# diaoenmao/HeteroFL-Computation-and-Communication-Efficient-Federated-Learning-for-Heterogeneous-Clients

Hardware: AMD Instinct MI355X
Metric: local-train samples/sec/node (higher is better)
Workload: dtype bfloat16; 1 GPU; model=resnet18, dataset=CIFAR10, control_name=1_100_0.1_iid_fix_a1-e1_bn_1_1, active_clients=10, local_epochs=5, global_batch=10, parallelism=client-dp1, engine=batched

## Files before the change

### heterofl_amd/ops/csrc/bindings.cpp

```cpp
#include <torch/extension.h>

std::vector<at::Tensor> bn_relu_fwd(at::Tensor x, at::Tensor gamma,
                                    at::Tensor beta, double eps);
std::vector<at::Tensor> bn_relu_bwd(at::Tensor dy, at::Tensor x,
                                    at::Tensor gamma, at::Tensor beta,
                                    at::Tensor mean, at::Tensor invstd);
std::vector<at::Tensor> gn_relu_fwd(at::Tensor x, at::Tensor gamma,
                                    at::Tensor beta, int64_t G, double eps);
std::vector<at::Tensor> gn_relu_bwd(at::Tensor dy, at::Tensor x,
                                    at::Tensor gamma, at::Tensor beta,
                                    at::Tensor mean, at::Tensor invstd,
                                    int64_t G);
std::vector<at::Tensor> masked_ce_fwd(at::Tensor scores, at::Tensor labels,
                                      at::Tensor mask, at::Tensor metrics);
at::Tensor masked_ce_bwd(at::Tensor scores, at::Tensor labels, at::Tensor mask,
                         at::Tensor up);
std::vector<at::Tensor> build_chunk_table(std::vector<at::Tensor> grads,
                                          std::vector<at::Tensor> params,
                                          std::vector<at::Tensor> bufs,
                                          int64_t R, int64_t chunk_elems,
                                          std::vector<at::Tensor> shadows);
void fill_chunk_table(at::Tensor blob, std::vector<at::Tensor> grads,
                      std::vector<at::Tensor> params,
                      std::vector<at::Tensor> bufs, int64_t R,
                      int64_t chunk_elems, std::vector<at::Tensor> shadows);
void clip_sgd_step(at::Tensor table_blob, int64_t n_chunks,
                   at::Tensor chunk_client, at::Tensor partials,
                   at::Tensor normsq, double max_norm, double lr,
                   double momentum, double weight_decay);
// ... 63 lines not shown
at::Tensor conv_pack_weight(at::Tensor w);
at::Tensor conv_fwd_large(at::Tensor x, at::Tensor packed, at::Tensor bias,
                          at::Tensor residual, int64_t stride, int64_t pad,
                          int64_t Cin, int64_t Cout, int64_t k);
at::Tensor bn_relu_infer(at::Tensor x, at::Tensor scale, at::Tensor shift);
std::vector<at::Tensor> eval_metrics(at::Tensor scores, at::Tensor labels,
                                     at::Tensor user_ptr,
                                     at::Tensor user_samples,
                                     at::Tensor label_mask);
at::Tensor lm_head_pack(at::Tensor w);
std::vector<at::Tensor> lm_head_ce(at::Tensor x, at::Tensor packed,
                                   at::Tensor bias, at::Tensor labels,
                                   at::Tensor vocab_mask, int64_t V,
                                   int64_t E, int64_t splits);
std::vector<at::Tensor> lm_head_topk(at::Tensor x, at::Tensor packed,
                                     at::Tensor bias, at::Tensor labels,
                                     at::Tensor vocab_mask, int64_t V,
                                     int64_t E, int64_t k, int64_t splits);
int64_t lm_head_topk_splits(int64_t M, int64_t V);

PYBIND11_MODULE(TORCH_EXTENSION_NAME, m) {
    m.def("bn_relu_fwd", &bn_relu_fwd, "fused sBN+ReLU forward");
    m.def("bn_relu_bwd", &bn_relu_bwd, "fused sBN+ReLU backward");
    m.def("gn_relu_fwd", &gn_relu_fwd, "fused GroupNorm+ReLU forward");
    m.def("gn_relu_bwd", &gn_relu_bwd, "fused GroupNorm+ReLU backward");
    m.def("masked_ce_fwd", &masked_ce_fwd, "batched masked CE forward");
    m.def("masked_ce_bwd", &masked_ce_bwd, "batched masked CE backward");
    m.def("build_chunk_table", &build_chunk_table,
          "build clip+SGD chunk table");
    m.def("clip_sgd_step", &clip_sgd_step, "fused per-client clip+SGD step");
    m.def("fill_chunk_table", &fill_chunk_table,
          "fill a preallocated chunk table post-capture");
    m.def("conv_fwd", &conv_fwd, "MFMA implicit-GEMM grouped conv forward");
    m.def("conv_bwd_data", &conv_bwd_data, "MFMA grouped conv backward-data");
    m.def("conv_bwd_weight", &conv_bwd_weight,
          "MFMA grouped conv backward-weight (fp32 out)");
    m.def("conv_plan", &conv_plan,
          "(route, split, dynamic LDS bytes) the conv launchers would take; "
          "launches nothing");
    m.def("conv_plan_variant", &conv_plan_variant,
          "name of the kernel the conv launcher would launch; launches "
          "nothing");
    m.def("mfma_probe", &mfma_probe, "16x16x32 bf16 MFMA layout probe");
    m.def("head_fwd", &head_fwd, "fused avgpool+per-client-linear forward");
    m.def("head_bwd", &head_bwd, "fused head backward");
    m.def("attn_fwd", &attn_fwd, "fused small-S attention forward");
// ... 44 lines not shown
```

### heterofl_amd/ops/csrc/clip_sgd.hip

```cpp
#include "common.h"

struct Chunk {
    const float* grad;
    float* param;
    float* buf;
    __hip_bfloat16* shadow;
    int len;
    int client;
};

__global__ void __launch_bounds__(256)
sqnorm_kernel(const Chunk* __restrict__ chunks,
              float* __restrict__ partials) {
    const Chunk ck = chunks[blockIdx.x];
    float s = 0.f;
    for (int i = threadIdx.x; i < ck.len; i += blockDim.x) {
        const float g = ck.grad[i];
        s += g * g;
    }
    __shared__ float scratch[256 / WAVE];
    for (int off = WAVE / 2; off > 0; off >>= 1) s += __shfl_down(s, off, WAVE);
    const int wid = threadIdx.x / WAVE;
    if ((threadIdx.x & (WAVE - 1)) == 0) scratch[wid] = s;
    __syncthreads();
// ... 11 lines not shown
    const int r = blockIdx.x;
    float s = 0.f;
    for (int i = threadIdx.x; i < n_chunks; i += 64)
        if (chunk_client[i] == r) s += partials[i];
    for (int off = WAVE / 2; off > 0; off >>= 1) s += __shfl_down(s, off, WAVE);
    if (threadIdx.x == 0) normsq[r] = s;
}

__global__ void __launch_bounds__(256)
clip_sgd_step_kernel(const Chunk* __restrict__ chunks,
                     const float* __restrict__ normsq, float max_norm,
                     float lr, float momentum, float weight_decay) {
    const Chunk ck = chunks[blockIdx.x];
    const float norm = sqrtf(normsq[ck.client]);
    const float scale = fminf(max_norm / (norm + 1e-6f), 1.f);
    for (int i = threadIdx.x; i < ck.len; i += blockDim.x) {
        const float p = ck.param[i];
        float g = ck.grad[i] * scale + weight_decay * p;
        const float b = momentum * ck.buf[i] + g;
        ck.buf[i] = b;
        const float pn = p - lr * b;
        ck.param[i] = pn;
        if (ck.shadow) ck.shadow[i] = __float2bfloat16(pn);
    }
}

#include <torch/extension.h>
#include <ATen/hip/HIPContext.h>

std::vector<at::Tensor> build_chunk_table(std::vector<at::Tensor> grads,
                                          std::vector<at::Tensor> params,
                                          std::vector<at::Tensor> bufs,
                                          int64_t R, int64_t chunk_elems,
                                          std::vector<at::Tensor> shadows) {
    std::vector<Chunk> host;
    for (size_t t = 0; t < grads.size(); ++t) {
        TORCH_CHECK(grads[t].is_contiguous() && params[t].is_contiguous() &&
                    bufs[t].is_contiguous());
        TORCH_CHECK(grads[t].scalar_type() == at::kFloat,
                    "clip_sgd expects fp32 master grads/params");
        const long numel = grads[t].numel();
        TORCH_CHECK(numel % R == 0);
        const long per = numel / R;
        const float* g = grads[t].data_ptr<float>();
        float* p = params[t].data_ptr<float>();
        float* b = bufs[t].data_ptr<float>();
// ... 55 lines not shown
                ck.grad = g + r * per + off;
                ck.param = p + r * per + off;
                ck.buf = b + r * per + off;
                ck.shadow = sh ? sh + r * per + off : nullptr;
                ck.len = (int)std::min((long)chunk_elems, per - off);
                ck.client = (int)r;
                host.push_back(ck);
            }
    }
    TORCH_CHECK((long)(host.size() * sizeof(Chunk)) == blob.numel(),
                "chunk table size changed");
    auto src = at::from_blob(host.data(), {(long)(host.size() * sizeof(Chunk))},
                             at::TensorOptions().dtype(at::kByte)).clone();
    blob.copy_(src, false);
}

void clip_sgd_step(at::Tensor table_blob, int64_t n_chunks,
                   at::Tensor chunk_client, at::Tensor partials,
                   at::Tensor normsq, double max_norm, double lr,
                   double momentum, double weight_decay) {
    auto stream = at::hip::getCurrentHIPStream();
    const Chunk* chunks = (const Chunk*)table_blob.data_ptr();
    const int R = (int)normsq.numel();
    hipLaunchKernelGGL(sqnorm_kernel, dim3((int)n_chunks), dim3(256), 0,
                       stream, chunks, partials.data_ptr<float>());
    hipLaunchKernelGGL(sqnorm_reduce_kernel, dim3(R), dim3(64), 0, stream,
                       partials.data_ptr<float>(),
                       chunk_client.data_ptr<int>(), (int)n_chunks,
                       normsq.data_ptr<float>());
    hipLaunchKernelGGL(clip_sgd_step_kernel, dim3((int)n_chunks), dim3(256), 0,
                       stream, chunks, normsq.data_ptr<float>(),
                       (float)max_norm, (float)lr, (float)momentum,
                       (float)weight_decay);
}
```

### heterofl_amd/ops/csrc/common.h

```cpp
#pragma once
#include <hip/hip_runtime.h>
#include <hip/hip_bf16.h>

#define WAVE 64

typedef __attribute__((ext_vector_type(4))) float f32x4;
typedef __attribute__((ext_vector_type(8))) __bf16 bf16x8;
typedef __attribute__((ext_vector_type(8))) unsigned short u16x8;

template <typename T>
__device__ __forceinline__ float ld_f32(const T* p) { return (float)*p; }
template <>
__device__ __forceinline__ float ld_f32<__hip_bfloat16>(const __hip_bfloat16* p) {
    return __bfloat162float(*p);
}

template <typename T>
__device__ __forceinline__ void st_f32(T* p, float v) { *p = (T)v; }
template <>
__device__ __forceinline__ void st_f32<__hip_bfloat16>(__hip_bfloat16* p, float v) {
    *p = __float2bfloat16(v);
}

__device__ __forceinline__ void block_reduce2(float& v1, float& v2, float* scratch) {
    for (int off = WAVE / 2; off > 0; off >>= 1) {
        v1 += __shfl_down(v1, off, WAVE);
        v2 += __shfl_down(v2, off, WAVE);
    }
    const int wid = threadIdx.x / WAVE;
    const int nw = blockDim.x / WAVE;
    if ((threadIdx.x & (WAVE - 1)) == 0) {
        scratch[2 * wid] = v1;
        scratch[2 * wid + 1] = v2;
    }
    __syncthreads();
    if (threadIdx.x < WAVE) {
        float a = (threadIdx.x < nw) ? scratch[2 * threadIdx.x] : 0.f;
        float b = (threadIdx.x < nw) ? scratch[2 * threadIdx.x + 1] : 0.f;
        for (int off = WAVE / 2; off > 0; off >>= 1) {
            a += __shfl_down(a, off, WAVE);
            b += __shfl_down(b, off, WAVE);
        }
        if (threadIdx.x == 0) { scratch[0] = a; scratch[1] = b; }
    }
// ... 6 lines not shown
```

### heterofl_amd/ops/csrc/conv_mfma.hip

```cpp
#include "common.h"

constexpr int BM = 64;
constexpr int BP = 64;
constexpr int BK = 32;
constexpr int LDK = BK + 8;

template <typename T>
__device__ __forceinline__ f32x4 mfma_tile(const T* a_row, const T* b_col,
                                           f32x4 acc);

template <>
__device__ __forceinline__ f32x4 mfma_tile<__hip_bfloat16>(
        const __hip_bfloat16* a_row, const __hip_bfloat16* b_col, f32x4 acc) {
    const int l = threadIdx.x & (WAVE - 1);
    const int kb = (l >> 4) * 8;
    bf16x8 a = *(const bf16x8*)(a_row + kb);
    bf16x8 b = *(const bf16x8*)(b_col + kb);
    return __builtin_amdgcn_mfma_f32_16x16x32_bf16(a, b, acc, 0, 0, 0);
}

template <>
__device__ __forceinline__ f32x4 mfma_tile<float>(const float* a_row,
                                                  const float* b_col,
                                                  f32x4 acc) {
// ... 227 lines not shown
            for (int r = 0; r < 4; ++r) {
                const int m = m0 + wm + fm * 16 + (l >> 4) * 4 + r;
                if (m < M && yb >= 0)
                    fwd_store(acc[fm][fp][r], yb + (long)m * OHW,
                              g * gm.Cout + m, bias, residual, y, partial,
                              slab, splitk);
            }
        }
}

template <typename T>
__global__ void __launch_bounds__(256)
conv_out_reduce_kernel(const float* __restrict__ partial,
                       const float* __restrict__ bias,
                       const T* __restrict__ residual, T* __restrict__ out,
                       long total, long chanstride, int nchan, int splitk) {
    const long i = (long)blockIdx.x * blockDim.x + threadIdx.x;
    if (i >= total) return;
    float v = 0.f;
    for (int sp = 0; sp < splitk; ++sp) v += partial[(long)sp * total + i];
    if (bias) v += bias[(i / chanstride) % nchan];
    if (residual) v += ld_f32(residual + i);
    st_f32(out + i, v);
}

template <typename T, typename TA, typename TB>
__global__ void __launch_bounds__(256)
conv_bwd_data_kernel(const T* __restrict__ dy, const float* __restrict__ w,
                     T* __restrict__ dx, float* __restrict__ partial,
                     ConvGeom gm, int splitk) {
    __shared__ TA a_lds[BM][LDK];
    __shared__ TB b_lds[BP][LDK];
    __shared__ int t_oh[BP], t_ow[BP];
    __shared__ long t_dybase[BP], t_xbase[BP];
    const TileCoord tc = tile_coord(gm.G);
    const int g = tc.g, sp = tc.sp;
    const int c0 = tc.row0, q0 = tc.col0;
    const int kk2 = gm.khw * gm.khw;
    const int J = gm.Cout * kk2;
    const int K = gm.Cin * kk2;
    const int HW = gm.H * gm.W;
    const int Q = gm.N * HW;
    const int OHW = gm.OH * gm.OW;
    const int tid = tc.tid, l = tc.l, wm = tc.wm, wp = tc.wp;

    if (tid < BP) {
// ... 333 lines not shown
    }
    float* slab = out + (long)sp * GK;
#pragma unroll
    for (int fm = 0; fm < 2; ++fm)
#pragma unroll
        for (int fp = 0; fp < 2; ++fp)
#pragma unroll
            for (int r = 0; r < 4; ++r) {
                const int m = m0 + wm + fm * 16 + (l >> 4) * 4 + r;
                const int k = k0 + wp + fp * 16 + (l & 15);
                if (m < M && k < K)
                    slab[(long)(g * gm.Cout + m) * K + k] = acc[fm][fp][r];
            }
}

__global__ void __launch_bounds__(256)
splitp_reduce_kernel(const float* __restrict__ partials,
                     float* __restrict__ dw, long GK, int splitp) {
    const long i = (long)blockIdx.x * blockDim.x + threadIdx.x;
    if (i >= GK) return;
    float s = 0.f;
    for (int sp = 0; sp < splitp; ++sp) s += partials[(long)sp * GK + i];
    dw[i] = s;
}


constexpr int WIN_CH = BK / 9 + 2;
constexpr int WIN_ROWS = 16;
constexpr int WIN_W = 40;

template <typename T, typename TA, typename TB>
__global__ void __launch_bounds__(256)
conv_fwd_staged_kernel(const T* __restrict__ x, const float* __restrict__ w,
                       const float* __restrict__ bias,
                       const T* __restrict__ residual, T* __restrict__ y,
                       float* __restrict__ partial, ConvGeom gm, int splitk) {
    __shared__ TA a_lds[BM][LDK];
    __shared__ TB b_lds[BP][LDK];
    __shared__ float win[WIN_CH][WIN_ROWS][WIN_W];
    const TileCoord tc = tile_coord(gm.G);
    const int g = tc.g, sp = tc.sp;
    const int m0 = tc.row0, p0 = tc.col0;
    const int kk2 = gm.khw * gm.khw;
    const int K = gm.Cin * kk2;
    const int M = gm.Cout;
    const int OHW = gm.OH * gm.OW;
// ... 1638 lines not shown
    std::string stem;
    if (direction == "fwd") {
        pl = plan_fwd(gm, (int)elem_size, fp8 != 0);
        stem = "conv_fwd";
    } else if (direction == "bwd_data") {
        pl = plan_bwd_data(gm, (int)elem_size, fp8 != 0);
        stem = pl.route == GATHER_S2 ? "conv_bwd_data_s2" : "conv_bwd_data";
    } else if (direction == "bwd_weight") {
        pl = plan_bwd_weight(gm, (int)elem_size, fp8 != 0);
        stem = "conv_bwd_weight";
    } else {
        TORCH_CHECK(false, "direction must be fwd, bwd_data or bwd_weight");
    }
    if (pl.route == RESIDENT) return stem + "_resident_kernel";
    if (pl.route == STAGED) return stem + "_staged_kernel";
    if (pl.tabled) return stem + "_tabled_kernel";
    return stem + (pl.fp8 ? "_kernel<fp8>" : "_kernel");
}

#define DISPATCH_CONV_FT(t, ...)                                              \
    if ((t) == at::kFloat) { using scalar_t = float; __VA_ARGS__; }           \
    else if ((t) == at::kBFloat16) { using scalar_t = __hip_bfloat16; __VA_ARGS__; } \
    else { TORCH_CHECK(false, "unsupported dtype"); }

template <typename T>
static auto fwd_kernel(const ConvPlan& pl) {
    if (pl.route == STAGED) return conv_fwd_staged_kernel<T, T, T>;
    if constexpr (std::is_same<T, __hip_bfloat16>::value)
        if (pl.fp8) return conv_fwd_kernel<T, e4m3, e4m3>;
    return conv_fwd_kernel<T, T, T>;
}
template <typename T>
static auto bwd_data_kernel(const ConvPlan& pl) {
    if (pl.route == STAGED) return conv_bwd_data_staged_kernel<T, T, T>;
    if constexpr (std::is_same<T, __hip_bfloat16>::value)
        if (pl.fp8) return conv_bwd_data_kernel<T, e4m3, e5m2>;
    return conv_bwd_data_kernel<T, T, T>;
}
template <typename T>
static auto bwd_data_s2_kernel(const ConvPlan& pl) {
    if constexpr (std::is_same<T, __hip_bfloat16>::value)
        if (pl.fp8) return conv_bwd_data_s2_kernel<T, e4m3, e5m2>;
    return conv_bwd_data_s2_kernel<T, T, T>;
}
template <typename T>
static auto bwd_weight_kernel(const ConvPlan& pl) {
// ... 29 lines not shown
                                 : nullptr;
        scalar_t* yp = (scalar_t*)y.data_ptr();
        if (pl.route == RESIDENT) {
            const int K = gm.Cin * gm.khw * gm.khw;
            const int flags =
                ((gm.W % (16 / esz) == 0 && aligned16(xp)) ? 1 : 0)
                | ((K % 4 == 0 && aligned16(wp)) ? 2 : 0);
            hipLaunchKernelGGL(conv_fwd_resident_kernel<scalar_t>, pl.grid,
                               dim3(256), pl.dyn_lds, stream, xp, wp, bp, rp,
                               yp, pp, gm, pl.split, pl.tab0, flags);
        } else if (pl.tabled) {
            const int K = gm.Cin * gm.khw * gm.khw;
            const int flags = (K % 4 == 0 && aligned16(wp)) ? 2 : 0;
            hipLaunchKernelGGL(conv_fwd_tabled_kernel<scalar_t>, pl.grid,
                               dim3(256), pl.tab_lds, stream, xp, wp, bp, rp, yp, pp,
                               gm, pl.split, flags);
        } else {
            hipLaunchKernelGGL(fwd_kernel<scalar_t>(pl), pl.grid, dim3(256),
                               0, stream, xp, wp, bp, rp, yp, pp, gm,
                               pl.split);
        }
        if (pl.split > 1) {
            const long total = y.numel();
            hipLaunchKernelGGL(conv_out_reduce_kernel<scalar_t>,
                               dim3((int)((total + 255) / 256)), dim3(256), 0,
                               stream, pp, bp, rp, yp, total,
                               (long)gm.OH * gm.OW, gm.G * gm.Cout, pl.split);
        }
    });
    return y;
}

at::Tensor conv_bwd_data(at::Tensor dy, at::Tensor w, int64_t groups,
                         int64_t stride, int64_t pad, int64_t H, int64_t W,
                         int64_t fp8) {
    TORCH_CHECK(dy.is_cuda() && w.is_contiguous());
    TORCH_CHECK(stride == 1 || stride == 2, "stride must be 1 or 2");
    auto dyc = dy.contiguous();
    const ConvGeom gm = conv_geom(groups, dy.size(0), w.size(1), H, W,
                                  w.size(0) / groups, w.size(2), stride, pad);
    TORCH_CHECK(dy.size(2) == gm.OH && dy.size(3) == gm.OW,
                "dy does not match the conv geometry");
    const int esz = (int)dy.element_size();
    const ConvPlan pl = plan_bwd_data(gm, esz, fp8 != 0);
    auto dx = at::empty({gm.N, gm.G * gm.Cin, gm.H, gm.W}, dy.options());
    at::Tensor partial;
    if (pl.split > 1)
        partial = at::empty({(long)pl.split * dx.numel()},
                            dy.options().dtype(at::kFloat));
    float* pp = pl.split > 1 ? partial.data_ptr<float>() : nullptr;
// ... 8 lines not shown
            hipLaunchKernelGGL(conv_bwd_data_resident_kernel<scalar_t>,
                               pl.grid, dim3(256), pl.dyn_lds, stream, dyp,
                               wp, dxp, pp, gm, pl.split, pl.tab0, pl.tab1,
                               flags);
        } else if (pl.tabled && pl.route == GATHER_S2) {
            hipLaunchKernelGGL(conv_bwd_data_s2_tabled_kernel<scalar_t>,
                               pl.grid, dim3(256), pl.tab_lds, stream, dyp, wp, dxp,
                               pp, gm, pl.split, pl.nyp);
        } else if (pl.tabled) {
            hipLaunchKernelGGL(conv_bwd_data_tabled_kernel<scalar_t>,
                               pl.grid, dim3(256), pl.tab_lds, stream, dyp, wp, dxp,
                               pp, gm, pl.split);
        } else if (pl.route == GATHER_S2) {
            hipLaunchKernelGGL(bwd_data_s2_kernel<scalar_t>(pl), pl.grid,
                               dim3(256), 0, stream, dyp, wp, dxp, pp, gm,
                               pl.split, pl.nyp);
        } else {
            hipLaunchKernelGGL(bwd_data_kernel<scalar_t>(pl), pl.grid,
                               dim3(256), 0, stream, dyp, wp, dxp, pp, gm,
                               pl.split);
        }
        if (pl.split > 1) {
            const long total = dx.numel();
            hipLaunchKernelGGL(conv_out_reduce_kernel<scalar_t>,
                               dim3((int)((total + 255) / 256)), dim3(256), 0,
                               stream, pp, nullptr, nullptr, dxp, total, 1L,
                               1, pl.split);
        }
    });
    return dx;
}

at::Tensor conv_bwd_weight(at::Tensor dy, at::Tensor x, int64_t groups,
                           int64_t stride, int64_t pad, int64_t khw,
                           int64_t fp8) {
    auto dyc = dy.contiguous();
    const ConvGeom gm = conv_geom(groups, x.size(0), x.size(1) / groups,
                                  x.size(2), x.size(3), dy.size(1) / groups,
                                  khw, stride, pad);
    TORCH_CHECK(dy.size(2) == gm.OH && dy.size(3) == gm.OW,
                "dy does not match the conv geometry");
    const int esz = (int)x.element_size();
    const ConvPlan pl = plan_bwd_weight(gm, esz, fp8 != 0);
    const long GK = (long)gm.G * gm.Cout * gm.Cin * gm.khw * gm.khw;
    auto dw = at::empty({(long)gm.G * gm.Cout, gm.Cin, gm.khw, gm.khw},
                        x.options().dtype(at::kFloat));
    at::Tensor partials;
    if (pl.split > 1)
        partials = at::empty({pl.split, GK}, x.options().dtype(at::kFloat));
    float* out = pl.split > 1 ? partials.data_ptr<float>()
// ... 3 lines not shown
        const scalar_t* dyp = (const scalar_t*)dyc.data_ptr();
        const scalar_t* xp = (const scalar_t*)x.data_ptr();
        if (pl.route == RESIDENT) {
            const int flags =
                ((gm.W % (16 / esz) == 0 && aligned16(xp)) ? 1 : 0)
                | (aligned16(dyp) ? 2 : 0);
            hipLaunchKernelGGL(conv_bwd_weight_resident_kernel<scalar_t>,
                               pl.grid, dim3(256), pl.dyn_lds, stream, dyp,
                               xp, out, gm, pl.split, flags);
        } else if (pl.tabled) {
            const int OHW = gm.OH * gm.OW;
            const int pchunk = cdiv(gm.N * OHW, pl.split);
            const int flags = (OHW % 8 == 0 && pchunk % 8 == 0
                               && aligned16(dyp)) ? 2 : 0;
            hipLaunchKernelGGL(conv_bwd_weight_tabled_kernel<scalar_t>,
                               pl.grid, dim3(256), 0, stream, dyp, xp, out,
                               gm, pl.split, flags);
        } else {
            hipLaunchKernelGGL(bwd_weight_kernel<scalar_t>(pl), pl.grid,
                               dim3(256), 0, stream, dyp, xp, out, gm,
                               pl.split);
        }
    });
    if (pl.split > 1)
        hipLaunchKernelGGL(splitp_reduce_kernel,
                           dim3((int)((GK + 255) / 256)), dim3(256), 0,
                           stream, out, dw.data_ptr<float>(), GK, pl.split);
    return dw;
}

__global__ void mfma_probe_kernel(const float* __restrict__ A,
                                  const float* __restrict__ B,
                                  float* __restrict__ D) {
    const int l = threadIdx.x;
    const int kb = (l >> 4) * 8;
    bf16x8 a, b;
#pragma unroll
    for (int j = 0; j < 8; ++j) {
        a[j] = (__bf16)A[(l & 15) * 32 + kb + j];
        b[j] = (__bf16)B[(kb + j) * 16 + (l & 15)];
    }
    f32x4 acc = {};
    acc = __builtin_amdgcn_mfma_f32_16x16x32_bf16(a, b, acc, 0, 0, 0);
#pragma unroll
    for (int r = 0; r < 4; ++r)
        D[((l >> 4) * 4 + r) * 16 + (l & 15)] = acc[r];
}

at::Tensor mfma_probe(at::Tensor A, at::Tensor B) {
    TORCH_CHECK(A.sizes() == at::IntArrayRef({16, 32}) &&
// ... 11 lines not shown
```

### heterofl_amd/ops/csrc/fused_norm.hip

```cpp
#include "common.h"

template <typename T, bool STAGE>
__global__ void __launch_bounds__(256)
bn_relu_fwd_kernel(const T* __restrict__ x, const float* __restrict__ gamma,
                   const float* __restrict__ beta, T* __restrict__ y,
                   float* __restrict__ mean_out, float* __restrict__ invstd_out,
                   int N, int C, int HW, float eps) {
    const int c = blockIdx.x;
    __shared__ float scratch[2 * 256 / WAVE];
    extern __shared__ __attribute__((aligned(16))) char smem[];
    T* stage = (T*)smem;
    float s1 = 0.f, s2 = 0.f;
    const long chan_off = (long)c * HW;
    const long samp_stride = (long)C * HW;
    for (int i = threadIdx.x; i < N * HW; i += blockDim.x) {
        const int n = i / HW, hw = i - n * HW;
        const T raw = x[n * samp_stride + chan_off + hw];
        if (STAGE) stage[i] = raw;
        const float v = (float)raw;
        s1 += v;
        s2 += v * v;
    }
    block_reduce2(s1, s2, scratch);
    const float inv_m = 1.f / (N * HW);
// ... 124 lines not shown
        s2 += d * xh;
    }
    block_reduce2(s1, s2, scratch);
    if (threadIdx.x == 0) {
        dbeta[c] = s1;
        dgamma[c] = s2;
    }
    const float inv_M = 1.f / (N * HW);
    const float k1 = s1 * inv_M, k2 = s2 * inv_M;
    const float gis = g * is;
    for (int i = threadIdx.x; i < N * HW; i += blockDim.x) {
        const int n = i / HW, hw = i - n * HW;
        const long off = n * samp_stride + chan_off + hw;
        float xh, d;
        if (STAGE) {
            xh = ((float)sx[i] - m) * is;
            d = (float)sd[i];
        } else {
            xh = (ld_f32(x + off) - m) * is;
            const float pre = xh * g + b;
            d = pre > 0.f ? ld_f32(dy + off) : 0.f;
        }
        st_f32(dx + off, gis * (d - k1 - xh * k2));
    }
}

template <typename T, bool STAGE>
__global__ void __launch_bounds__(256)
gn_relu_fwd_kernel(const T* __restrict__ x, const float* __restrict__ gamma,
                   const float* __restrict__ beta, T* __restrict__ y,
                   float* __restrict__ mean_out, float* __restrict__ invstd_out,
                   int N, int C, int HW, int G, float eps) {
    const int ng = blockIdx.x;
    const int n = ng / G, j = ng - n * G;
    const int cpg = C / G;
    __shared__ float scratch[2 * 256 / WAVE];
    extern __shared__ __attribute__((aligned(16))) char smem[];
    T* stage = (T*)smem;
    const long base = (long)n * C * HW + (long)j * cpg * HW;
    const int M = cpg * HW;
    float s1 = 0.f, s2 = 0.f;
    for (int i = threadIdx.x; i < M; i += blockDim.x) {
        const T raw = x[base + i];
        if (STAGE) stage[i] = raw;
        const float v = (float)raw;
        s1 += v;
// ... 61 lines not shown
        s2 += d * g * xh;
    }
    block_reduce2(s1, s2, scratch);
    const float inv_M = 1.f / M;
    const float k1 = s1 * inv_M, k2 = s2 * inv_M;
    for (int i = threadIdx.x; i < M; i += blockDim.x) {
        const int c = j * cpg + i / HW;
        const float g = gamma ? gamma[c] : 1.f;
        const float b = beta ? beta[c] : 0.f;
        const float xh = (ld_f32(x + base + i) - m) * is;
        const float pre = xh * g + b;
        const float d = pre > 0.f ? ld_f32(dy + base + i) : 0.f;
        st_f32(dx + base + i, is * (d * g - k1 - xh * k2));
    }
}

#include <torch/extension.h>
#include <ATen/hip/HIPContext.h>

#define DISPATCH_FT(t, ...)                                                   \
    if ((t) == at::kFloat) { using scalar_t = float; __VA_ARGS__; }           \
    else if ((t) == at::kBFloat16) { using scalar_t = __hip_bfloat16; __VA_ARGS__; } \
    else { TORCH_CHECK(false, "unsupported dtype"); }

std::vector<at::Tensor> bn_relu_fwd(at::Tensor x, at::Tensor gamma,
                                    at::Tensor beta, double eps) {
    TORCH_CHECK(x.is_cuda() && x.is_contiguous());
    const int N = x.size(0), C = x.size(1);
    const int HW = x.numel() / (N * C);
    auto y = at::empty_like(x);
    auto opts = x.options().dtype(at::kFloat);
    auto mean = at::empty({C}, opts);
    auto invstd = at::empty({C}, opts);
    auto stream = at::hip::getCurrentHIPStream();
    const long stage_bytes = (long)N * HW * x.element_size();
    const long M = (long)N * HW;
    if (M > 64 * 1024) {
        const int S = std::max(1, std::min(N, (4096 + C - 1) / C));
        auto partials = at::empty({(long)C * S * 2}, opts);
        auto scale_shift = at::empty({2L * C}, opts);
        DISPATCH_FT(x.scalar_type(), {
            hipLaunchKernelGGL(bn_sums_kernel<scalar_t>, dim3(C, S),
                               dim3(256), 0, stream,
                               (const scalar_t*)x.data_ptr(),
                               partials.data_ptr<float>(), N, C, HW, S);
            hipLaunchKernelGGL(bn_finalize_kernel,
                               dim3((C + 255) / 256), dim3(256), 0, stream,
                               partials.data_ptr<float>(),
                               gamma.defined() ? gamma.data_ptr<float>()
                                               : nullptr,
                               beta.defined() ? beta.data_ptr<float>()
                                              : nullptr,
                               mean.data_ptr<float>(),
                               invstd.data_ptr<float>(),
                               scale_shift.data_ptr<float>(), C, S,
                               (float)(1.0 / M), (float)eps);
            hipLaunchKernelGGL(bn_apply_relu_kernel<scalar_t>, dim3(C, S),
                               dim3(256), 0, stream,
                               (const scalar_t*)x.data_ptr(),
                               scale_shift.data_ptr<float>(),
                               (scalar_t*)y.data_ptr(), N, C, HW, S);
        });
        return {y, mean, invstd};
    }
    DISPATCH_FT(x.scalar_type(), {
        if (stage_bytes <= 64 * 1024)
            hipLaunchKernelGGL((bn_relu_fwd_kernel<scalar_t, true>), dim3(C),
                               dim3(256), (int)stage_bytes, stream,
                               (const scalar_t*)x.data_ptr(),
                               gamma.defined() ? gamma.data_ptr<float>()
                                               : nullptr,
                               beta.defined() ? beta.data_ptr<float>()
                                              : nullptr,
                               (scalar_t*)y.data_ptr(),
                               mean.data_ptr<float>(),
                               invstd.data_ptr<float>(), N, C, HW,
                               (float)eps);
        else
            hipLaunchKernelGGL((bn_relu_fwd_kernel<scalar_t, false>), dim3(C),
                               dim3(256), 0, stream,
                               (const scalar_t*)x.data_ptr(),
                               gamma.defined() ? gamma.data_ptr<float>()
                                               : nullptr,
                               beta.defined() ? beta.data_ptr<float>()
                                              : nullptr,
                               (scalar_t*)y.data_ptr(),
                               mean.data_ptr<float>(),
                               invstd.data_ptr<float>(), N, C, HW,
                               (float)eps);
    });
    return {y, mean, invstd};
}

std::vector<at::Tensor> bn_relu_bwd(at::Tensor dy, at::Tensor x,
                                    at::Tensor gamma, at::Tensor beta,
                                    at::Tensor mean, at::Tensor invstd) {
    const int N = x.size(0), C = x.size(1);
    const int HW = x.numel() / (N * C);
    auto dx = at::empty_like(x);
    auto opts = x.options().dtype(at::kFloat);
    auto dgamma = at::empty({C}, opts);
    auto dbeta = at::empty({C}, opts);
    auto dyc = dy.contiguous();
    auto stream = at::hip::getCurrentHIPStream();
    const long stage_bytes = 2L * N * (x.numel() / (N * C)) * x.element_size();
    DISPATCH_FT(x.scalar_type(), {
        if (stage_bytes <= 64 * 1024)
            hipLaunchKernelGGL((bn_relu_bwd_kernel<scalar_t, true>), dim3(C),
                               dim3(256), (int)stage_bytes, stream,
                               (const scalar_t*)dyc.data_ptr(),
                               (const scalar_t*)x.data_ptr(),
                               gamma.defined() ? gamma.data_ptr<float>()
                                               : nullptr,
                               beta.defined() ? beta.data_ptr<float>()
                                              : nullptr,
                               mean.data_ptr<float>(),
                               invstd.data_ptr<float>(),
                               (scalar_t*)dx.data_ptr(),
                               dgamma.data_ptr<float>(),
                               dbeta.data_ptr<float>(), N, C, HW);
        else
            hipLaunchKernelGGL((bn_relu_bwd_kernel<scalar_t, false>), dim3(C),
                               dim3(256), 0, stream,
                               (const scalar_t*)dyc.data_ptr(),
                               (const scalar_t*)x.data_ptr(),
                               gamma.defined() ? gamma.data_ptr<float>()
                                               : nullptr,
                               beta.defined() ? beta.data_ptr<float>()
                                              : nullptr,
                               mean.data_ptr<float>(),
                               invstd.data_ptr<float>(),
                               (scalar_t*)dx.data_ptr(),
                               dgamma.data_ptr<float>(),
                               dbeta.data_ptr<float>(), N, C, HW);
    });
    return {dx, dgamma, dbeta};
}

std::vector<at::Tensor> gn_relu_fwd(at::Tensor x, at::Tensor gamma,
                                    at::Tensor beta, int64_t G, double eps) {
    TORCH_CHECK(x.is_cuda() && x.is_contiguous());
    const int N = x.size(0), C = x.size(1);
    const int HW = x.numel() / (N * C);
    TORCH_CHECK(C % G == 0, "channels not divisible by groups");
    auto y = at::empty_like(x);
    auto opts = x.options().dtype(at::kFloat);
    auto mean = at::empty({N * G}, opts);
    auto invstd = at::empty({N * G}, opts);
    auto stream = at::hip::getCurrentHIPStream();
    const long gsb = ((long)C / G) * (x.numel() / (N * C)) * x.element_size();
    DISPATCH_FT(x.scalar_type(), {
        if (gsb <= 64 * 1024)
            hipLaunchKernelGGL((gn_relu_fwd_kernel<scalar_t, true>),
                               dim3(N * G), dim3(256), (int)gsb, stream,
                               (const scalar_t*)x.data_ptr(),
                               gamma.defined() ? gamma.data_ptr<float>()
                                               : nullptr,
// ... 68 lines not shown
```

### heterofl_amd/ops/fused.py

```python
import torch
import torch.nn.functional as F

from . import require_native, use_native, large_conv_enabled


class _FusedNormReLU(torch.autograd.Function):

    @staticmethod
    def forward(ctx, x, weight, bias, kind, groups, eps):
        ext = require_native()
        x = x.contiguous()
        if kind == 'bn':
            y, mean, invstd = ext.bn_relu_fwd(x, weight, bias, eps)
        else:
            y, mean, invstd = ext.gn_relu_fwd(x, weight, bias, groups, eps)
        ctx.save_for_backward(x, weight, bias, mean, invstd)
        ctx.kind = kind
        ctx.groups = groups
        return y

    @staticmethod
    def backward(ctx, dy):
        ext = require_native()
        x, weight, bias, mean, invstd = ctx.saved_tensors
        if ctx.kind == 'bn':
            dx, dgamma, dbeta = ext.bn_relu_bwd(dy, x, weight, bias, mean,
                                                invstd)
        else:
            dx, dgamma, dbeta = ext.gn_relu_bwd(dy, x, weight, bias, mean,
                                                invstd, ctx.groups)
        return dx, dgamma, dbeta, None, None, None


def fused_norm_relu(x, weight, bias, kind, groups=1, eps=1e-5):
    return _FusedNormReLU.apply(x, weight, bias, kind, groups, eps)


def eager_scaler_norm_relu(x, weight, bias, kind, groups, rate, eps=1e-5):
    if rate != 1.0:
        x = x / rate
    if kind == 'bn':
        x = F.batch_norm(x, None, None, weight, bias, training=True, eps=eps)
    else:
        x = F.group_norm(x, groups, weight, bias, eps=eps)
    return F.relu(x)


class _FusedMaskedCE(torch.autograd.Function):

    @staticmethod
    def forward(ctx, scores, labels, mask, metrics):
        ext = require_native()
        scores = scores.contiguous().float()
        (losses,) = ext.masked_ce_fwd(
            scores, labels.contiguous(),
            mask if mask is not None else torch.Tensor(),
            metrics if metrics is not None else torch.Tensor())
        ctx.save_for_backward(scores, labels,
# ... 571 lines not shown
```

Baseline: 24820 samples/s.

## Vectorize memory-bound streaming kernels: clip-SGD, split-K reductions, BN+ReLU

Adds 16-byte vectorized variants of several bandwidth-bound kernels: an unrolled squared-norm kernel and float4 clip+SGD step, float4 split-K output and weight-gradient reductions with fused bias and residual, and vectorized staged BN+ReLU forward/backward. A route selector picks the vector path when pointers and sizes are aligned and the HETEROFL_STREAM_VEC environment variable does not disable it. The goal is fewer memory instructions and better load-level parallelism in elementwise and reduction passes, at the cost of more code paths and alignment-dependent dispatch. A new binding reports which BN route would be taken.

```diff
diff --git a/heterofl_amd/ops/csrc/bindings.cpp b/heterofl_amd/ops/csrc/bindings.cpp
--- a/heterofl_amd/ops/csrc/bindings.cpp
+++ b/heterofl_amd/ops/csrc/bindings.cpp
@@ -5,6 +5,8 @@
 std::vector<at::Tensor> bn_relu_bwd(at::Tensor dy, at::Tensor x,
                                     at::Tensor gamma, at::Tensor beta,
                                     at::Tensor mean, at::Tensor invstd);
+std::string bn_relu_route(const std::string& direction, int64_t N, int64_t C,
+                          int64_t HW, int64_t elem_size, bool aligned);
 std::vector<at::Tensor> gn_relu_fwd(at::Tensor x, at::Tensor gamma,
                                     at::Tensor beta, int64_t G, double eps);
 std::vector<at::Tensor> gn_relu_bwd(at::Tensor dy, at::Tensor x,
@@ -114,6 +116,9 @@
 PYBIND11_MODULE(TORCH_EXTENSION_NAME, m) {
     m.def("bn_relu_fwd", &bn_relu_fwd, "fused sBN+ReLU forward");
     m.def("bn_relu_bwd", &bn_relu_bwd, "fused sBN+ReLU backward");
+    m.def("bn_relu_route", &bn_relu_route,
+          "name of the kernel route bn_relu_fwd / bn_relu_bwd would take; "
+          "launches nothing");
     m.def("gn_relu_fwd", &gn_relu_fwd, "fused GroupNorm+ReLU forward");
     m.def("gn_relu_bwd", &gn_relu_bwd, "fused GroupNorm+ReLU backward");
     m.def("masked_ce_fwd", &masked_ce_fwd, "batched masked CE forward");
diff --git a/heterofl_amd/ops/csrc/clip_sgd.hip b/heterofl_amd/ops/csrc/clip_sgd.hip
--- a/heterofl_amd/ops/csrc/clip_sgd.hip
+++ b/heterofl_amd/ops/csrc/clip_sgd.hip
@@ -57,6 +57,106 @@
         const float pn = p - lr * b;
         ck.param[i] = pn;
         if (ck.shadow) ck.shadow[i] = __float2bfloat16(pn);
+    }
+}
+
+constexpr int SQ_U = 16;
+
+__global__ void __launch_bounds__(256)
+sqnorm_unrolled_kernel(const Chunk* __restrict__ chunks,
+                       float* __restrict__ partials) {
+    const Chunk ck = chunks[blockIdx.x];
+    const gptr<const float> grad = as_global(ck.grad);
+    float s = 0.f;
+    int i = threadIdx.x;
+    for (; i + 256 * (SQ_U - 1) < ck.len; i += 256 * SQ_U) {
+        float g[SQ_U];
+#pragma unroll
+        for (int u = 0; u < SQ_U; ++u) g[u] = grad[i + 256 * u];
+#pragma unroll
+        for (int u = 0; u < SQ_U; ++u) s = __fmaf_rn(g[u], g[u], s);
+    }
+    for (; i < ck.len; i += 256) {
+        const float g = grad[i];
+        s = __fmaf_rn(g, g, s);
+    }
+    __shared__ float scratch[256 / WAVE];
+    for (int off = WAVE / 2; off > 0; off >>= 1) s += __shfl_down(s, off, WAVE);
+    const int wid = threadIdx.x / WAVE;
+    if ((threadIdx.x & (WAVE - 1)) == 0) scratch[wid] = s;
+    __syncthreads();
+    if (threadIdx.x == 0) {
+        float t = 0.f;
+        for (int w = 0; w < blockDim.x / WAVE; ++w) t += scratch[w];
+        partials[blockIdx.x] = t;
+    }
+}
+
+constexpr int STEP_U = 2;
+
+__device__ __forceinline__ void sgd_elem(float& p, float gr, float& bf,
+                                         float scale, float lr,
+                                         float momentum, float weight_decay) {
+    const float g = __fmaf_rn(weight_decay, p, gr * scale);
+    const float b = __fmaf_rn(momentum, bf, g);
+    bf = b;
+    p = __fmaf_rn(-lr, b, p);
+}
+
+__global__ void __launch_bounds__(256)
+clip_sgd_step_vec_kernel(const Chunk* __restrict__ chunks,
+                         const float* __restrict__ normsq, float max_norm,
+                         float lr, float momentum, float weight_decay) {
+    const Chunk ck = chunks[blockIdx.x];
+    const float norm = sqrtf(normsq[ck.client]);
+    const float scale = fminf(max_norm / (norm + 1e-6f), 1.f);
+    const unsigned long bits = (unsigned long)ck.grad | (unsigned long)ck.param
+                               | (unsigned long)ck.buf;
+    const bool vec = (bits & 15) == 0 && ((unsigned long)ck.shadow & 7) == 0
+                     && (ck.len & 3) == 0;
+    if (!vec) {
+        for (int i = threadIdx.x; i < ck.len; i += blockDim.x) {
+            float p = ck.param[i], b = ck.buf[i];
+            sgd_elem(p, ck.grad[i], b, scale, lr, momentum, weight_decay);
+            ck.buf[i] = b;
+            ck.param[i] = p;
+            if (ck.shadow) ck.shadow[i] = __float2bfloat16(p);
+        }
+        return;
+    }
+    const gptr<const f32x4> g4 = (gptr<const f32x4>)as_global(ck.grad);
+    const gptr<f32x4> p4 = (gptr<f32x4>)as_global(ck.param);
+    const gptr<f32x4> b4 = (gptr<f32x4>)as_global(ck.buf);
+    const gptr<u32x2> s4 = (gptr<u32x2>)as_global(ck.shadow);
+    const int n4 = ck.len >> 2;
+    for (int i0 = threadIdx.x; i0 < n4; i0 += 256 * STEP_U) {
+        f32x4 g[STEP_U], p[STEP_U], b[STEP_U];
+#pragma unroll
+        for (int u = 0; u < STEP_U; ++u) {
+            const int i = i0 + 256 * u < n4 ? i0 + 256 * u : i0;
+            g[u] = g4[i];
+            p[u] = p4[i];
+            b[u] = b4[i];
+        }
+#pragma unroll
+        for (int u = 0; u < STEP_U; ++u) {
+            const int i = i0 + 256 * u;
+            if (i < n4) {
+                float pe[4], be[4];
+#pragma unroll
+                for (int e = 0; e < 4; ++e) {
+                    pe[e] = p[u][e];
+                    be[e] = b[u][e];
+                    sgd_elem(pe[e], g[u][e], be[e], scale, lr, momentum,
+                             weight_decay);
+                }
+                b4[i] = f32x4{be[0], be[1], be[2], be[3]};
+                p4[i] = f32x4{pe[0], pe[1], pe[2], pe[3]};
+                if (ck.shadow)
+                    s4[i] = u32x2{pack_bf16x2(pe[0], pe[1]),
+                                  pack_bf16x2(pe[2], pe[3])};
+            }
+        }
     }
 }
 
@@ -158,14 +258,17 @@
     auto stream = at::hip::getCurrentHIPStream();
     const Chunk* chunks = (const Chunk*)table_blob.data_ptr();
     const int R = (int)normsq.numel();
-    hipLaunchKernelGGL(sqnorm_kernel, dim3((int)n_chunks), dim3(256), 0,
-                       stream, chunks, partials.data_ptr<float>());
+    const bool vec = stream_vec_on();
+    hipLaunchKernelGGL(vec ? sqnorm_unrolled_kernel : sqnorm_kernel,
+                       dim3((int)n_chunks), dim3(256), 0, stream, chunks,
+                       partials.data_ptr<float>());
     hipLaunchKernelGGL(sqnorm_reduce_kernel, dim3(R), dim3(64), 0, stream,
                        partials.data_ptr<float>(),
                        chunk_client.data_ptr<int>(), (int)n_chunks,
                        normsq.data_ptr<float>());
-    hipLaunchKernelGGL(clip_sgd_step_kernel, dim3((int)n_chunks), dim3(256), 0,
-                       stream, chunks, normsq.data_ptr<float>(),
+    hipLaunchKernelGGL(vec ? clip_sgd_step_vec_kernel : clip_sgd_step_kernel,
+                       dim3((int)n_chunks), dim3(256), 0, stream, chunks,
+                       normsq.data_ptr<float>(),
                        (float)max_norm, (float)lr, (float)momentum,
                        (float)weight_decay);
 }
diff --git a/heterofl_amd/ops/csrc/common.h b/heterofl_amd/ops/csrc/common.h
--- a/heterofl_amd/ops/csrc/common.h
+++ b/heterofl_amd/ops/csrc/common.h
@@ -1,6 +1,7 @@
 #pragma once
 #include <hip/hip_runtime.h>
 #include <hip/hip_bf16.h>
+#include <cstdlib>
 
 #define WAVE 64
 
@@ -20,6 +21,52 @@
 template <>
 __device__ __forceinline__ void st_f32<__hip_bfloat16>(__hip_bfloat16* p, float v) {
     *p = __float2bfloat16(v);
+}
+
+template <typename T>
+__device__ __forceinline__ void unpack16(const uint4& r, float* f) {
+    f[0] = __uint_as_float(r.x);
+    f[1] = __uint_as_float(r.y);
+    f[2] = __uint_as_float(r.z);
+    f[3] = __uint_as_float(r.w);
+}
+template <>
+__device__ __forceinline__ void unpack16<__hip_bfloat16>(const uint4& r,
+                                                         float* f) {
+    const unsigned w[4] = {r.x, r.y, r.z, r.w};
+#pragma unroll
+    for (int i = 0; i < 4; ++i) {
+        f[2 * i] = __uint_as_float(w[i] << 16);
+        f[2 * i + 1] = __uint_as_float(w[i] & 0xffff0000u);
+    }
+}
+__device__ __forceinline__ unsigned pack_bf16x2(float lo, float hi) {
+    return (unsigned)__bfloat16_as_ushort(__float2bfloat16(lo))
+           | ((unsigned)__bfloat16_as_ushort(__float2bfloat16(hi)) << 16);
+}
+template <typename T>
+__device__ __forceinline__ uint4 pack16(const float* f) {
+    return make_uint4(__float_as_uint(f[0]), __float_as_uint(f[1]),
+                      __float_as_uint(f[2]), __float_as_uint(f[3]));
+}
+template <>
+__device__ __forceinline__ uint4 pack16<__hip_bfloat16>(const float* f) {
+    return make_uint4(pack_bf16x2(f[0], f[1]), pack_bf16x2(f[2], f[3]),
+                      pack_bf16x2(f[4], f[5]), pack_bf16x2(f[6], f[7]));
+}
+
+template <typename T>
+using gptr = __attribute__((address_space(1))) T*;
+template <typename T>
+__device__ __forceinline__ gptr<T> as_global(T* p) { return (gptr<T>)p; }
+typedef __attribute__((ext_vector_type(2))) unsigned u32x2;
+
+static inline bool stream_vec_on() {
+    const char* e = std::getenv("HETEROFL_STREAM_VEC");
+    return !(e && e[0] == '0');
+}
+static inline bool ptr_aligned(const void* p, unsigned long bytes) {
+    return (reinterpret_cast<unsigned long>(p) & (bytes - 1)) == 0;
 }
 
 __device__ __forceinline__ void block_reduce2(float& v1, float& v2, float* scratch) {
diff --git a/heterofl_amd/ops/csrc/conv_mfma.hip b/heterofl_amd/ops/csrc/conv_mfma.hip
--- a/heterofl_amd/ops/csrc/conv_mfma.hip
+++ b/heterofl_amd/ops/csrc/conv_mfma.hip
@@ -273,6 +273,91 @@
     if (bias) v += bias[(i / chanstride) % nchan];
     if (residual) v += ld_f32(residual + i);
     st_f32(out + i, v);
+}
+
+constexpr int RED_U = 8;
+
+__device__ __forceinline__ float4 sum_slabs_f4(const float4* __restrict__ p,
+                                               long stride4, int split) {
+    float4 s = make_float4(0.f, 0.f, 0.f, 0.f);
+    int sp = 0;
+    for (; sp + RED_U <= split; sp += RED_U) {
+        float4 a[RED_U];
+#pragma unroll
+        for (int u = 0; u < RED_U; ++u) a[u] = p[(sp + u) * stride4];
+#pragma unroll
+        for (int u = 0; u < RED_U; ++u) {
+            s.x += a[u].x;
+            s.y += a[u].y;
+            s.z += a[u].z;
+            s.w += a[u].w;
+        }
+    }
+    if (sp + 4 <= split) {
+        float4 a[4];
+#pragma unroll
+        for (int u = 0; u < 4; ++u) a[u] = p[(sp + u) * stride4];
+#pragma unroll
+        for (int u = 0; u < 4; ++u) {
+            s.x += a[u].x;
+            s.y += a[u].y;
+            s.z += a[u].z;
+            s.w += a[u].w;
+        }
+        sp += 4;
+    }
+    if (sp + 2 <= split) {
+        const float4 a0 = p[sp * stride4], a1 = p[(sp + 1) * stride4];
+        s.x += a0.x; s.y += a0.y; s.z += a0.z; s.w += a0.w;
+        s.x += a1.x; s.y += a1.y; s.z += a1.z; s.w += a1.w;
+        sp += 2;
+    }
+    if (sp < split) {
+        const float4 a0 = p[sp * stride4];
+        s.x += a0.x; s.y += a0.y; s.z += a0.z; s.w += a0.w;
+    }
+    return s;
+}
+
+template <typename T, int BIAS, typename IDX>
+__global__ void __launch_bounds__(256)
+conv_out_reduce_vec_kernel(const float* __restrict__ partial,
+                           const float* __restrict__ bias,
+                           const T* __restrict__ residual,
+                           T* __restrict__ out, long total, long chanstride,
+                           int nchan, int splitk) {
+    const long i4 = (long)blockIdx.x * blockDim.x + threadIdx.x;
+    const long total4 = total >> 2;
+    if (i4 >= total4) return;
+    const float4 s = sum_slabs_f4((const float4*)partial + i4, total4, splitk);
+    float v[4] = {s.x, s.y, s.z, s.w};
+    if (BIAS == 1) {
+        const float bv =
+            bias[((IDX)(i4 * 4) / (IDX)chanstride) % (IDX)nchan];
+#pragma unroll
+        for (int e = 0; e < 4; ++e) v[e] += bv;
+    } else if (BIAS == 2) {
+#pragma unroll
+        for (int e = 0; e < 4; ++e)
+            v[e] += bias[((IDX)(i4 * 4 + e) / (IDX)chanstride) % (IDX)nchan];
+    }
+    if (sizeof(T) == 4) {
+        if (residual) {
+            const float4 r = ((const float4*)residual)[i4];
+            v[0] += r.x; v[1] += r.y; v[2] += r.z; v[3] += r.w;
+        }
+        ((float4*)out)[i4] = make_float4(v[0], v[1], v[2], v[3]);
+    } else {
+        if (residual) {
+            const uint2 r = ((const uint2*)residual)[i4];
+            v[0] += __uint_as_float(r.x << 16);
+            v[1] += __uint_as_float(r.x & 0xffff0000u);
+            v[2] += __uint_as_float(r.y << 16);
+            v[3] += __uint_as_float(r.y & 0xffff0000u);
+        }
+        ((uint2*)out)[i4] = make_uint2(pack_bf16x2(v[0], v[1]),
+                                       pack_bf16x2(v[2], v[3]));
+    }
 }
 
 template <typename T, typename TA, typename TB>
@@ -652,6 +737,16 @@
     float s = 0.f;
     for (int sp = 0; sp < splitp; ++sp) s += partials[(long)sp * GK + i];
     dw[i] = s;
+}
+
+__global__ void __launch_bounds__(256)
+splitp_reduce_vec_kernel(const float* __restrict__ partials,
+                         float* __restrict__ dw, long GK, int splitp) {
+    const long i4 = (long)blockIdx.x * blockDim.x + threadIdx.x;
+    const long GK4 = GK >> 2;
+    if (i4 >= GK4) return;
+    ((float4*)dw)[i4] = sum_slabs_f4((const float4*)partials + i4, GK4,
+                                     splitp);
 }
 
 
@@ -2336,6 +2431,32 @@
     if ((t) == at::kFloat) { using scalar_t = float; __VA_ARGS__; }           \
     else if ((t) == at::kBFloat16) { using scalar_t = __hip_bfloat16; __VA_ARGS__; } \
     else { TORCH_CHECK(false, "unsupported dtype"); }
+
+template <typename T>
+static void launch_out_reduce(hipStream_t stream, const float* pp,
+                              const float* bp, const T* rp, T* yp, long total,
+                              long chanstride, int nchan, int split) {
+    const bool vec = stream_vec_on() && total % 4 == 0 &&
+                     ptr_aligned(pp, 16) && ptr_aligned(yp, 4 * sizeof(T)) &&
+                     (!rp || ptr_aligned(rp, 4 * sizeof(T)));
+    if (!vec) {
+        hipLaunchKernelGGL(conv_out_reduce_kernel<T>,
+                           dim3((int)((total + 255) / 256)), dim3(256), 0,
+                           stream, pp, bp, rp, yp, total, chanstride, nchan,
+                           split);
+        return;
+    }
+    const bool wide = total >= (1L << 31);
+    auto kern = !bp ? conv_out_reduce_vec_kernel<T, 0, int>
+                : chanstride % 4 == 0
+                    ? (wide ? conv_out_reduce_vec_kernel<T, 1, long>
+                            : conv_out_reduce_vec_kernel<T, 1, int>)
+                    : (wide ? conv_out_reduce_vec_kernel<T, 2, long>
+                            : conv_out_reduce_vec_kernel<T, 2, int>);
+    hipLaunchKernelGGL(kern, dim3((int)((total / 4 + 255) / 256)), dim3(256),
+                       0, stream, pp, bp, rp, yp, total, chanstride, nchan,
+                       split);
+}
 
 template <typename T>
 static auto fwd_kernel(const ConvPlan& pl) {
@@ -2411,10 +2532,9 @@
         }
         if (pl.split > 1) {
             const long total = y.numel();
-            hipLaunchKernelGGL(conv_out_reduce_kernel<scalar_t>,
-                               dim3((int)((total + 255) / 256)), dim3(256), 0,
-                               stream, pp, bp, rp, yp, total,
-                               (long)gm.OH * gm.OW, gm.G * gm.Cout, pl.split);
+            launch_out_reduce<scalar_t>(stream, pp, bp, rp, yp, total,
+                                        (long)gm.OH * gm.OW, gm.G * gm.Cout,
+                                        pl.split);
         }
     });
     return y;
@@ -2469,10 +2589,8 @@
         }
         if (pl.split > 1) {
             const long total = dx.numel();
-            hipLaunchKernelGGL(conv_out_reduce_kernel<scalar_t>,
-                               dim3((int)((total + 255) / 256)), dim3(256), 0,
-                               stream, pp, nullptr, nullptr, dxp, total, 1L,
-                               1, pl.split);
+            launch_out_reduce<scalar_t>(stream, pp, nullptr, nullptr, dxp,
+                                        total, 1L, 1, pl.split);
         }
     });
     return dx;
@@ -2522,10 +2640,19 @@
                                pl.split);
         }
     });
-    if (pl.split > 1)
-        hipLaunchKernelGGL(splitp_reduce_kernel,
-                           dim3((int)((GK + 255) / 256)), dim3(256), 0,
-                           stream, out, dw.data_ptr<float>(), GK, pl.split);
+    if (pl.split > 1) {
+        if (stream_vec_on() && GK % 4 == 0 && aligned16(out) &&
+            aligned16(dw.data_ptr<float>()))
+            hipLaunchKernelGGL(splitp_reduce_vec_kernel,
+                               dim3((int)((GK / 4 + 255) / 256)), dim3(256),
+                               0, stream, out, dw.data_ptr<float>(), GK,
+                               pl.split);
+        else
+            hipLaunchKernelGGL(splitp_reduce_kernel,
+                               dim3((int)((GK + 255) / 256)), dim3(256), 0,
+                               stream, out, dw.data_ptr<float>(), GK,
+                               pl.split);
+    }
     return dw;
 }
 
diff --git a/heterofl_amd/ops/csrc/fused_norm.hip b/heterofl_amd/ops/csrc/fused_norm.hip
--- a/heterofl_amd/ops/csrc/fused_norm.hip
+++ b/heterofl_amd/ops/csrc/fused_norm.hip
@@ -170,6 +170,172 @@
             d = pre > 0.f ? ld_f32(dy + off) : 0.f;
         }
         st_f32(dx + off, gis * (d - k1 - xh * k2));
+    }
+}
+
+constexpr int BN_VEC_U = 4;
+
+struct RowWalk {
+    int n, j, dn, dj, vpr;
+    __device__ __forceinline__ RowWalk(int v, int vpr_) : vpr(vpr_) {
+        n = v / vpr;
+        j = v - n * vpr;
+        dn = 256 / vpr;
+        dj = 256 - dn * vpr;
+    }
+    __device__ __forceinline__ void step() {
+        j += dj;
+        n += dn;
+        if (j >= vpr) {
+            j -= vpr;
+            ++n;
+        }
+    }
+};
+
+template <typename T>
+__global__ void __launch_bounds__(256)
+bn_relu_fwd_vec_kernel(const T* __restrict__ x,
+                       const float* __restrict__ gamma,
+                       const float* __restrict__ beta, T* __restrict__ y,
+                       float* __restrict__ mean_out,
+                       float* __restrict__ invstd_out, int N, int C, int HW,
+                       float eps) {
+    constexpr int V = 16 / sizeof(T);
+    const int c = blockIdx.x;
+    __shared__ float scratch[2 * 256 / WAVE];
+    extern __shared__ __attribute__((aligned(16))) char smem[];
+    const T* stage = (const T*)smem;
+    uint4* stage4 = (uint4*)smem;
+    const int M = N * HW;
+    const int nvec = M / V;
+    const long samp_stride = (long)C * HW;
+    const T* xc = x + (long)c * HW;
+    T* yc = y + (long)c * HW;
+    RowWalk rw(threadIdx.x, HW / V);
+    for (int v0 = threadIdx.x; v0 < nvec; v0 += 256 * BN_VEC_U) {
+        uint4 r[BN_VEC_U];
+        const long off0 = rw.n * samp_stride + rw.j * V;
+#pragma unroll
+        for (int u = 0; u < BN_VEC_U; ++u) {
+            const long off = v0 + u * 256 < nvec
+                                 ? rw.n * samp_stride + rw.j * V : off0;
+            r[u] = *(const uint4*)(xc + off);
+            rw.step();
+        }
+#pragma unroll
+        for (int u = 0; u < BN_VEC_U; ++u)
+            if (v0 + u * 256 < nvec) stage4[v0 + u * 256] = r[u];
+    }
+    __syncthreads();
+    float s1 = 0.f, s2 = 0.f;
+#pragma unroll 8
+    for (int i = threadIdx.x; i < M; i += 256) {
+        const float v = (float)stage[i];
+        s1 += v;
+        s2 += v * v;
+    }
+    block_reduce2(s1, s2, scratch);
+    const float inv_m = 1.f / (N * HW);
+    const float mean = s1 * inv_m;
+    const float var = fmaxf(s2 * inv_m - mean * mean, 0.f);
+    const float invstd = rsqrtf(var + eps);
+    if (threadIdx.x == 0) {
+        mean_out[c] = mean;
+        invstd_out[c] = invstd;
+    }
+    const float g = gamma ? gamma[c] : 1.f;
+    const float b = beta ? beta[c] : 0.f;
+    const float scale = invstd * g;
+    const float shift = b - mean * scale;
+    RowWalk ww(threadIdx.x, HW / V);
+    for (int v = threadIdx.x; v < nvec; v += 256) {
+        float f[V];
+        unpack16<T>(stage4[v], f);
+#pragma unroll
+        for (int e = 0; e < V; ++e) f[e] = fmaxf(f[e] * scale + shift, 0.f);
+        *(uint4*)(yc + ww.n * samp_stride + ww.j * V) = pack16<T>(f);
+        ww.step();
+    }
+}
+
+template <typename T>
+__global__ void __launch_bounds__(256)
+bn_relu_bwd_vec_kernel(const T* __restrict__ dy, const T* __restrict__ x,
+                       const float* __restrict__ gamma,
+                       const float* __restrict__ beta,
+                       const float* __restrict__ mean,
+                       const float* __restrict__ invstd, T* __restrict__ dx,
+                       float* __restrict__ dgamma, float* __restrict__ dbeta,
+                       int N, int C, int HW) {
+    constexpr int V = 16 / sizeof(T);
+    const int c = blockIdx.x;
+    __shared__ float scratch[2 * 256 / WAVE];
+    extern __shared__ __attribute__((aligned(16))) char smem[];
+    const int M = N * HW;
+    const int nvec = M / V;
+    const T* sx = (const T*)smem;
+    const T* sd = sx + M;
+    uint4* sx4 = (uint4*)sx;
+    uint4* sd4 = (uint4*)sd;
+    const long samp_stride = (long)C * HW;
+    const T* xc = x + (long)c * HW;
+    const T* dyc = dy + (long)c * HW;
+    T* dxc = dx + (long)c * HW;
+    const float m = mean[c], is = invstd[c];
+    const float g = gamma ? gamma[c] : 1.f;
+    const float b = beta ? beta[c] : 0.f;
+    RowWalk rw(threadIdx.x, HW / V);
+    for (int v0 = threadIdx.x; v0 < nvec; v0 += 256 * BN_VEC_U) {
+        uint4 rx[BN_VEC_U], rd[BN_VEC_U];
+        const long off0 = rw.n * samp_stride + rw.j * V;
+#pragma unroll
+        for (int u = 0; u < BN_VEC_U; ++u) {
+            const long off = v0 + u * 256 < nvec
+                                 ? rw.n * samp_stride + rw.j * V : off0;
+            rx[u] = *(const uint4*)(xc + off);
+            rd[u] = *(const uint4*)(dyc + off);
+            rw.step();
+        }
+#pragma unroll
+        for (int u = 0; u < BN_VEC_U; ++u)
+            if (v0 + u * 256 < nvec) {
+                sx4[v0 + u * 256] = rx[u];
+                sd4[v0 + u * 256] = rd[u];
+            }
+    }
+    __syncthreads();
+    float s1 = 0.f, s2 = 0.f;
+#pragma unroll 8
+    for (int i = threadIdx.x; i < M; i += 256) {
+        const float xh = ((float)sx[i] - m) * is;
+        const float pre = xh * g + b;
+        const float d = pre > 0.f ? ld_f32(sd + i) : 0.f;
+        s1 += d;
+        s2 += d * xh;
+    }
+    block_reduce2(s1, s2, scratch);
+    if (threadIdx.x == 0) {
+        dbeta[c] = s1;
+        dgamma[c] = s2;
+    }
+    const float inv_M = 1.f / (N * HW);
+    const float k1 = s1 * inv_M, k2 = s2 * inv_M;
+    const float gis = g * is;
+    RowWalk ww(threadIdx.x, HW / V);
+    for (int v = threadIdx.x; v < nvec; v += 256) {
+        float fx[V], fd[V];
+        unpack16<T>(sx4[v], fx);
+        unpack16<T>(sd4[v], fd);
+#pragma unroll
+        for (int e = 0; e < V; ++e) {
+            const float xh = (fx[e] - m) * is;
+            const float pre = xh * g + b;
+            const float d = pre > 0.f ? fd[e] : 0.f;
+            fd[e] = gis * (d - k1 - xh * k2);
+        }
+        *(uint4*)(dxc + ww.n * samp_stride + ww.j * V) = pack16<T>(fd);
+        ww.step();
     }
 }
 
@@ -277,6 +443,26 @@
     if ((t) == at::kFloat) { using scalar_t = float; __VA_ARGS__; }           \
     else if ((t) == at::kBFloat16) { using scalar_t = __hip_bfloat16; __VA_ARGS__; } \
     else { TORCH_CHECK(false, "unsupported dtype"); }
+
+enum BnRoute { BN_VEC, BN_STAGED, BN_DIRECT, BN_SPLIT3 };
+
+static BnRoute bn_route(bool bwd, long N, long HW, int esz, bool aligned) {
+    const long M = N * HW;
+    if (!bwd && M > 64 * 1024) return BN_SPLIT3;
+    if ((bwd ? 2 : 1) * M * esz > 64 * 1024) return BN_DIRECT;
+    if (stream_vec_on() && aligned && (HW * esz) % 16 == 0) return BN_VEC;
+    return BN_STAGED;
+}
+
+std::string bn_relu_route(const std::string& direction, int64_t N, int64_t C,
+                          int64_t HW, int64_t elem_size, bool aligned) {
+    TORCH_CHECK(direction == "fwd" || direction == "bwd",
+                "direction must be fwd or bwd");
+    (void)C;
+    static const char* names[] = {"vec", "staged", "direct", "split3"};
+    return names[bn_route(direction == "bwd", N, HW, (int)elem_size,
+                          aligned)];
+}
 
 std::vector<at::Tensor> bn_relu_fwd(at::Tensor x, at::Tensor gamma,
                                     at::Tensor beta, double eps) {
@@ -318,31 +504,20 @@
         });
         return {y, mean, invstd};
     }
+    const BnRoute route = bn_route(false, N, HW, (int)x.element_size(),
+                                   ptr_aligned(x.data_ptr(), 16) &&
+                                       ptr_aligned(y.data_ptr(), 16));
+    const float* gp = gamma.defined() ? gamma.data_ptr<float>() : nullptr;
+    const float* bp = beta.defined() ? beta.data_ptr<float>() : nullptr;
     DISPATCH_FT(x.scalar_type(), {
-        if (stage_bytes <= 64 * 1024)
-            hipLaunchKernelGGL((bn_relu_fwd_kernel<scalar_t, true>), dim3(C),
-                               dim3(256), (int)stage_bytes, stream,
-                               (const scalar_t*)x.data_ptr(),
-                               gamma.defined() ? gamma.data_ptr<float>()
-                                               : nullptr,
-                               beta.defined() ? beta.data_ptr<float>()
-                                              : nullptr,
-                               (scalar_t*)y.data_ptr(),
-                               mean.data_ptr<float>(),
-                               invstd.data_ptr<float>(), N, C, HW,
-                               (float)eps);
-        else
-            hipLaunchKernelGGL((bn_relu_fwd_kernel<scalar_t, false>), dim3(C),
-                               dim3(256), 0, stream,
-                               (const scalar_t*)x.data_ptr(),
-                               gamma.defined() ? gamma.data_ptr<float>()
-                                               : nullptr,
-                               beta.defined() ? beta.data_ptr<float>()
-                                              : nullptr,
-                               (scalar_t*)y.data_ptr(),
-                               mean.data_ptr<float>(),
-                               invstd.data_ptr<float>(), N, C, HW,
-                               (float)eps);
+        auto kern = route == BN_VEC ? bn_relu_fwd_vec_kernel<scalar_t>
+                    : route == BN_STAGED ? bn_relu_fwd_kernel<scalar_t, true>
+                                         : bn_relu_fwd_kernel<scalar_t, false>;
+        hipLaunchKernelGGL(kern, dim3(C), dim3(256),
+                           route == BN_DIRECT ? 0 : (int)stage_bytes, stream,
+                           (const scalar_t*)x.data_ptr(), gp, bp,
+                           (scalar_t*)y.data_ptr(), mean.data_ptr<float>(),
+                           invstd.data_ptr<float>(), N, C, HW, (float)eps);
     });
     return {y, mean, invstd};
 }
@@ -359,35 +534,23 @@
     auto dyc = dy.contiguous();
     auto stream = at::hip::getCurrentHIPStream();
     const long stage_bytes = 2L * N * (x.numel() / (N * C)) * x.element_size();
+    const BnRoute route = bn_route(true, N, HW, (int)x.element_size(),
+                                   ptr_aligned(x.data_ptr(), 16) &&
+                                       ptr_aligned(dyc.data_ptr(), 16) &&
+                                       ptr_aligned(dx.data_ptr(), 16));
+    const float* gp = gamma.defined() ? gamma.data_ptr<float>() : nullptr;
+    const float* bp = beta.defined() ? beta.data_ptr<float>() : nullptr;
     DISPATCH_FT(x.scalar_type(), {
-        if (stage_bytes <= 64 * 1024)
-            hipLaunchKernelGGL((bn_relu_bwd_kernel<scalar_t, true>), dim3(C),
-                               dim3(256), (int)stage_bytes, stream,
-                               (const scalar_t*)dyc.data_ptr(),
-                               (const scalar_t*)x.data_ptr(),
-                               gamma.defined() ? gamma.data_ptr<float>()
-                                               : nullptr,
-                               beta.defined() ? beta.data_ptr<float>()
-                                              : nullptr,
-                               mean.data_ptr<float>(),
-                               invstd.data_ptr<float>(),
-                               (scalar_t*)dx.data_ptr(),
-                               dgamma.data_ptr<float>(),
-                               dbeta.data_ptr<float>(), N, C, HW);
-        else
-            hipLaunchKernelGGL((bn_relu_bwd_kernel<scalar_t, false>), dim3(C),
-                               dim3(256), 0, stream,
-                               (const scalar_t*)dyc.data_ptr(),
-                               (const scalar_t*)x.data_ptr(),
-                               gamma.defined() ? gamma.data_ptr<float>()
-                                               : nullptr,
-                               beta.defined() ? beta.data_ptr<float>()
-                                              : nullptr,
-                               mean.data_ptr<float>(),
-                               invstd.data_ptr<float>(),
-                               (scalar_t*)dx.data_ptr(),
-                               dgamma.data_ptr<float>(),
-                               dbeta.data_ptr<float>(), N, C, HW);
+        auto kern = route == BN_VEC ? bn_relu_bwd_vec_kernel<scalar_t>
+                    : route == BN_STAGED ? bn_relu_bwd_kernel<scalar_t, true>
+                                         : bn_relu_bwd_kernel<scalar_t, false>;
+        hipLaunchKernelGGL(kern, dim3(C), dim3(256),
+                           route == BN_DIRECT ? 0 : (int)stage_bytes, stream,
+                           (const scalar_t*)dyc.data_ptr(),
+                           (const scalar_t*)x.data_ptr(), gp, bp,
+                           mean.data_ptr<float>(), invstd.data_ptr<float>(),
+                           (scalar_t*)dx.data_ptr(), dgamma.data_ptr<float>(),
+                           dbeta.data_ptr<float>(), N, C, HW);
     });
     return {dx, dgamma, dbeta};
 }
diff --git a/heterofl_amd/ops/fused.py b/heterofl_amd/ops/fused.py
--- a/heterofl_amd/ops/fused.py
+++ b/heterofl_amd/ops/fused.py
@@ -34,6 +34,11 @@
 
 def fused_norm_relu(x, weight, bias, kind, groups=1, eps=1e-5):
     return _FusedNormReLU.apply(x, weight, bias, kind, groups, eps)
+
+
+def bn_relu_route(direction, N, C, HW, elem_size, aligned=True):
+    ext = require_native()
+    return ext.bn_relu_route(direction, N, C, HW, elem_size, aligned)
 
 
 def eager_scaler_norm_relu(x, weight, bias, kind, groups, rate, eps=1e-5):
```

Measured after the change: 29200 samples/s (median of 6 runs). 1.18x the previous value.
